# Chlumsky/msdfgen

Hardware: AMD Instinct MI355X
Metric: MSDF glyphs/sec (64x64, fp32) (higher is better)
Workload: dtype f64

## Files before the change

### msdfgen_amd/csrc/msdf_capi.hip

```cpp

#include <hip/hip_runtime.h>

#include <atomic>
#include <chrono>
#include <condition_variable>
#include <cmath>
#include <cstdarg>
#include <cstdio>
#include <cstdlib>
#include <cstring>
#include <deque>
#include <functional>
#include <memory>
#include <mutex>
#include <string>
#include <thread>
#include <vector>

#include <sched.h>

#include "msdf_kernels.hpp"
#include "msdf_single.hpp"

using namespace msdfhip;
// ... 18 lines not shown

static long long nowNsEarly() { return std::chrono::duration_cast<std::chrono::nanoseconds>(std::chrono::steady_clock::now().time_since_epoch()).count(); }

struct Tuning {
    size_t resLdsBudget;
    long persistentRounds;
    bool serialClasses;
    int querySlotCap, queryLpcContours;
    bool hasQueryLds;
    bool hasQueryPolicy;
    int qpEdgeCost, qpMaxEdges, qpMinCount, qpWideMaxEdges;
    float qpWideLoad, qpWideMeanCount;
    size_t signCap;
    bool pipelineTrace;
    int microbatch;
    int queryStatic;
    int queryGridSteps;
    int queryBatch;
    bool noArgPayloadSingle;
    bool noZeroCopySingle;
    bool noFusedSingle;
    double shareGridFactor;
    long persistentGrid;
    long shortRounds;
    long smallLaunchTiles;
    char devices[256];
    int smallMaxEdges;
    int ldsClassTpw;
    int pipelineDepth;
    bool prepLargeTier;
    int hostThreads;
    long singleSpinLimit;
    bool singleVerbose;
};
std::atomic<const Tuning *> gTuning(NULL);
std::mutex gTuningMutex;
std::vector<Tuning *> gTuningTables;

void readTuning() {
    Tuning &t = *new Tuning;
    const char *env;
    t.resLdsBudget = (env = getenv("MSDFHIP_RES_LDS_BUDGET")) ? (size_t) atol(env) : (size_t) 10*1024;
    t.persistentRounds = (env = getenv("MSDFHIP_PERSISTENT_ROUNDS")) ? atol(env) : 8;
    t.serialClasses = getenv("MSDFHIP_SERIAL_CLASSES") != NULL;
    t.querySlotCap = 160, t.queryLpcContours = 24;
    t.hasQueryLds = (env = getenv("MSDFHIP_QUERY_LDS")) != NULL;
    if (env)
        sscanf(env, "%d,%d", &t.querySlotCap, &t.queryLpcContours);
    t.qpEdgeCost = 150, t.qpMaxEdges = 48, t.qpMinCount = 0x7fffffff, t.qpWideMaxEdges = 128, t.qpWideLoad = 4e8f, t.qpWideMeanCount = 24.f;
    t.hasQueryPolicy = (env = getenv("MSDFHIP_QUERY_POLICY")) != NULL;
    if (env)
        sscanf(env, "%d,%d,%d,%d,%f,%f", &t.qpEdgeCost, &t.qpMaxEdges, &t.qpMinCount, &t.qpWideMaxEdges, &t.qpWideLoad, &t.qpWideMeanCount);
    t.signCap = (env = getenv("MSDFHIP_SIGN_CAP")) ? (size_t) atol(env) : (size_t) 192;
    if (t.signCap < 3)
        t.signCap = 3;
    t.pipelineTrace = getenv("MSDFHIP_PIPELINE_TRACE") != NULL;
    t.microbatch = (env = getenv("MSDFHIP_MICROBATCH")) ? atoi(env) : 256;
    if (t.microbatch < 1)
        t.microbatch = 1;
    t.devices[0] = 0;
    t.queryStatic = (env = getenv("MSDFHIP_QUERY_STATIC")) ? atoi(env) : 2;
    t.queryGridSteps = (env = getenv("MSDFHIP_QUERY_GRID")) ? atoi(env) : 16;
    t.queryBatch = (env = getenv("MSDFHIP_QUERY_BATCH")) && atoi(env) > 0 ? atoi(env) : 1;
    t.noFusedSingle = getenv("MSDFHIP_NO_FUSED_SINGLE") != NULL;
    t.noZeroCopySingle = getenv("MSDFHIP_NO_ZERO_COPY_SINGLE") != NULL;
    t.noArgPayloadSingle = getenv("MSDFHIP_NO_ARG_PAYLOAD_SINGLE") != NULL;
    t.shortRounds = (env = getenv("MSDFHIP_SHORT_ROUNDS")) ? atol(env) : 4;
    t.persistentGrid = (env = getenv("MSDFHIP_PERSISTENT_GRID")) ? atol(env) : 0;
    t.shareGridFactor = (env = getenv("MSDFHIP_SHARE_GRID")) ? atof(env) : 1.33;
    t.smallLaunchTiles = (env = getenv("MSDFHIP_SMALL_LAUNCH_TILES")) ? atol(env) : 8192;
    if ((env = getenv("MSDFHIP_DEVICES")))
        snprintf(t.devices, sizeof(t.devices), "%s", env);
    t.smallMaxEdges = (env = getenv("MSDFHIP_SMALL_MAX_EDGES")) && atoi(env) > 0 ? atoi(env) : 128;
    t.ldsClassTpw = (env = getenv("MSDFHIP_LDS_CLASS_TPW")) && atoi(env) == 1 ? 1 : 4;
    t.pipelineDepth = (env = getenv("MSDFHIP_PIPELINE_DEPTH")) && atoi(env) >= 1 && atoi(env) <= 3 ? atoi(env) : 2;
    t.prepLargeTier = getenv("MSDFHIP_PREP_LARGE_TIER") != NULL;
    t.hostThreads = (env = getenv("MSDFHIP_HOST_THREADS")) && atoi(env) > 0 ? atoi(env) : 0;
    t.singleSpinLimit = (env = getenv("MSDFHIP_SINGLE_SPIN_LIMIT")) && atol(env) > 0 ? atol(env) : 0;
    t.singleVerbose = getenv("MSDFHIP_SINGLE_VERBOSE") != NULL;
    gTuningTables.push_back(&t);
    gTuning.store(&t, std::memory_order_release);
}

const Tuning &tuning() {
    const Tuning *t = gTuning.load(std::memory_order_acquire);
    if (!t) {
        std::lock_guard<std::mutex> lock(gTuningMutex);
        if (!gTuning.load(std::memory_order_acquire))
            readTuning();
        t = gTuning.load(std::memory_order_acquire);
    }
    return *t;
}

std::atomic<unsigned long long> gRouteCounts[MSDFHIP_ROUTE_COUNT];

inline void countRoute(int route) { gRouteCounts[route].fetch_add(1, std::memory_order_relaxed); }

#define HIPCHK(expr) do { hipError_t e_ = (expr); if (e_ != hipSuccess) { (void) hipGetLastError(); return fail(MSDFHIP_ERR_HIP, "%s failed: %s (%s:%d)", #expr, hipGetErrorString(e_), __FILE__, __LINE__); } } while (0)

int ensureDevice(int dev = -1) {
    if (gDevice.load() < 0) {
        int rc = msdfhip_init(0);
        if (rc != MSDFHIP_OK)
            return rc;
    }
    if (dev < 0)
        dev = gDevice.load();
    else if (dev != gDevice.load()) {
        static std::atomic<unsigned long long> checked(0);
        if (dev >= 64 || !((checked.load()>>dev)&1ull)) {
            hipDeviceProp_t prop;
// ... 661 lines not shown
        } else if (rc == MSDFHIP_OK)
            rc = counted(launchDistance<SEL, false, false>(b, dGlyphs, w, h, dst, toScratch, simple, sOne, b->dBucket, b->nOne), MSDFHIP_ROUTE_DIST_ONE_QUAD);
    }
    hipError_t joinError = hipSuccess;
    if (sRest != stream) {
        hipError_t e = hipEventRecord(b->joinEvent[0], sRest);
        if (e == hipSuccess)
            e = hipStreamWaitEvent(stream, b->joinEvent[0], 0);
        joinError = e != hipSuccess ? e : joinError;
    }
    if (sOne != stream) {
        hipError_t e = hipEventRecord(b->joinEvent[1], sOne);
        if (e == hipSuccess)
            e = hipStreamWaitEvent(stream, b->joinEvent[1], 0);
        joinError = e != hipSuccess ? e : joinError;
    }
    rc = aheadRc != MSDFHIP_OK ? aheadRc : rc;
    if (joinError != hipSuccess) {
        (void) hipGetLastError();
        if (sRest != stream)
            (void) hipStreamSynchronize(sRest);
        if (sOne != stream)
            (void) hipStreamSynchronize(sOne);
        if (rc == MSDFHIP_OK)
            rc = fail(MSDFHIP_ERR_HIP, "joining the glyph-class streams failed: %s", hipGetErrorString(joinError));
    }
    if (rc == MSDFHIP_OK && nHuge > 0)
        rc = launchUnculled<SEL, true>(b, dGlyphs, w, h, dst, toScratch, stream, b->dBucket+nCulled, nHuge);
    return rc;
}

size_t candidateRecords(int nGlyphs, size_t texelsPerGlyph) { return ecHeaderRecords(nGlyphs)+(size_t) nGlyphs*ecSegment(texelsPerGlyph); }
size_t offsetRecords(int nGlyphs) { return (ecOffsetInts(nGlyphs)*sizeof(int)+sizeof(EcCandidate)-1)/sizeof(EcCandidate); }
size_t deferredRecords(int nGlyphs, size_t texelsPerGlyph, int nEdges) {
    return candidateRecords(nGlyphs, texelsPerGlyph)+offsetRecords(nGlyphs)+((size_t) (nEdges > 0 ? nEdges : 1)*2*sizeof(int)+sizeof(EcCandidate)-1)/sizeof(EcCandidate);
}

int ensureDeferred(const MsdfHipBatch *b, size_t cap, EcCandidate **out) {
    std::lock_guard<std::mutex> lock(b->scratchMutex);
    if (b->deferredCap < cap) {
        if (b->dDeferred)
            hipFree(b->dDeferred);
        b->dDeferred = NULL;
        b->deferredCap = 0;
        HIPCHK(hipMalloc((void **) &b->dDeferred, cap*sizeof(EcCandidate)));
        b->deferredCap = cap;
    }
    if (!b->dEcParams)
        HIPCHK(hipMalloc((void **) &b->dEcParams, sizeof(EcGlyphParams)*(size_t) (b->nGlyphs > b->glyphCap ? b->nGlyphs : b->glyphCap > 0 ? b->glyphCap : 1)));
    *out = b->dDeferred;
    return MSDFHIP_OK;
}

template <int N, bool OVERLAP>
unsigned queryResidentBlocks(int device, size_t lds) {
    enum { LDS_STEP = 2048, LDS_STEPS = 81 };
    static std::atomic<int> cache[LDS_STEPS];
    const size_t step = (lds+LDS_STEP-1)/LDS_STEP;
    if (step >= LDS_STEPS)
        return 0;
    int v = cache[step].load();
    if (!v) {
        int perCu = 0;
        if (hipOccupancyMaxActiveBlocksPerMultiprocessor(&perCu, reinterpret_cast<const void *>(k_ec_query<N, OVERLAP>), WAVE, step*LDS_STEP) != hipSuccess) {
            (void) hipGetLastError();
            perCu = 0;
        }
        v = perCu > 0 ? perCu*residentSlots(device) : -1;
// ... 46 lines not shown
    bool wideSlots = false;
    if (b->nGlyphs < 256 && !tuning().hasQueryLds) {
        const int wide = b->maxEdges < 1024 ? (b->maxEdges > 0 ? b->maxEdges : 1) : 1024;
        const int wideMerged = b->maxContours < wide ? (b->maxContours > 0 ? b->maxContours : 1) : wide;
        if ((size_t) b->maxContours*sizeof(double)+(size_t) (wide+wideMerged)*sizeof(PBSlot) <= (size_t) 64*1024 && wide > slotCap)
            slotCap = wide, wideSlots = true;
    }
    EcQueryPolicy lpcMaxContours;
    lpcMaxContours.lpcMaxContours = b->maxContours < lpcContoursWanted ? b->maxContours : lpcContoursWanted;
    lpcMaxContours.lpcEdgeCost = tuning().qpEdgeCost, lpcMaxContours.lpcMaxEdges = tuning().qpMaxEdges, lpcMaxContours.lpcMinCount = tuning().qpMinCount;
    lpcMaxContours.wideMaxEdges = tuning().qpWideMaxEdges, lpcMaxContours.wideLoad = tuning().qpWideLoad, lpcMaxContours.wideMeanCount = tuning().qpWideMeanCount;
    lpcMaxContours.gridSteps = tuning().queryGridSteps;
    const size_t resLanes = OVERLAP ? (size_t) (lpcMaxContours.lpcMaxContours > 0 ? lpcMaxContours.lpcMaxContours : 1)*WAVE*sizeof(double) : 0;
    const int slotOffset = OVERLAP ? (b->maxContours > 0 ? b->maxContours : 1) : 0;
    const int mergedCap = b->maxContours < slotCap ? (b->maxContours > 0 ? b->maxContours : 1) : slotCap;
    const size_t coopLds = (size_t) slotOffset*sizeof(double)+(size_t) (slotCap+mergedCap)*sizeof(PBSlot);
    const size_t queryLds = resLanes > coopLds ? resLanes : coopLds;
    const size_t fastLds = ecFastLdsBytes(b->maxEdges, N);
    if (GRES && queryLds > (size_t) gLdsLimit.load() && fastLds <= (size_t) gLdsLimit.load()) {
        if (paramsOnly)
            return MSDFHIP_OK;
        hipLaunchKernelGGL((k_ec_slow<N, OVERLAP, GRES>), dim3(slowGrid), dim3(WAVE), slowLds, stream, viewOf(b), dGlyphs, w, h, src, out, stencil, cfg,
                           (const EcCandidate *) NULL, 0u, 0, gres, gresStride);
        HIPCHK(hipGetLastError());
        countRoute(MSDFHIP_ROUTE_EC_SLOW_ALL);
        return MSDFHIP_OK;
    }
    if (fastLds > (size_t) gLdsLimit.load() || queryLds > (size_t) gLdsLimit.load())
        return fail(MSDFHIP_ERR_TOO_COMPLEX, "a glyph has %d contours / %d edges: the error-correction pass needs %zu B of LDS per wavefront, device limit is %d B",
                    b->maxContours, b->maxEdges, fastLds > queryLds ? fastLds : queryLds, gLdsLimit.load());
    rc = setLds(k_ec_query<N, OVERLAP>, queryLds);
    if (rc != MSDFHIP_OK)
        return rc;
    rc = setLds(k_ec_fast<N>, fastLds);
    if (rc != MSDFHIP_OK)
        return rc;
    int *offsets = reinterpret_cast<int *>(deferred+candidateRecords(b->nGlyphs, (size_t) w*h));
    int *corners = reinterpret_cast<int *>(deferred+candidateRecords(b->nGlyphs, (size_t) w*h)+offsetRecords(b->nGlyphs));
    const size_t wanted = allTexels/512;
    unsigned queryBlocks = (unsigned) (wanted < 64 ? 64 : wanted > 8192 ? 8192 : wanted);
    const bool staticDeal = tuning().queryStatic != 0;
    if (staticDeal) {
        const unsigned resident = queryResidentBlocks<N, OVERLAP>(b->device, queryLds);
        if (resident && queryBlocks > resident)
            queryBlocks = resident;
    }
    if (!call.ecParamsQueued)
        hipLaunchKernelGGL(k_ec_params, dim3((unsigned) b->nGlyphs), dim3(WAVE), 0, stream, b->dEcParams, viewOf(b), dGlyphs, cfg,
                           reinterpret_cast<unsigned *>(deferred), corners, offsets+ecSizesAt(b->nGlyphs));
    const int *ecOrder = NULL;
    rc = ensureEcOrder(b, &ecOrder, stream);
    if (rc != MSDFHIP_OK)
        return rc;
    if (paramsOnly) {
        HIPCHK(hipGetLastError());
        call.ecParamsQueued = true;
        return MSDFHIP_OK;
    }
    hipLaunchKernelGGL((k_ec_fast<N>), dim3(blocks), dim3(WAVE), fastLds, stream, viewOf(b), dGlyphs, w, h, tilesX, tiles, src, out, stencil, cfg,
                       (const EcGlyphParams *) b->dEcParams, deferred, seg, b->maxEdges, (const int *) corners);
    hipLaunchKernelGGL(k_ec_scan, dim3(1), dim3(1024), 0, stream, b->nGlyphs, reinterpret_cast<const unsigned *>(deferred), seg, offsets, lpcMaxContours, ecOrder);
    hipLaunchKernelGGL((k_ec_query<N, OVERLAP>), dim3(queryBlocks), dim3(WAVE), queryLds, stream, b->nGlyphs, b->dGlyphContourOffsets, b->dContourOffsets,
                       (const EdgeRec *) viewOf(b).recs, viewOf(b).windings, dGlyphs, w, h, src, out, stencil, cfg,
                       (const EcGlyphParams *) b->dEcParams, (const EcCandidate *) deferred, seg, (const int *) offsets, offsets+2*(size_t) b->nGlyphs+2, tuning().queryBatch, slotCap, slotOffset, lpcMaxContours,
                       call.overflowOut, ecOrder, staticDeal ? (tuning().queryStatic == 2 ? 5 : 1) : 0);
    if (call.overflowOut)
        call.overflowMirrored = true;
    else
        hipLaunchKernelGGL((k_ec_slow<N, OVERLAP, GRES>), dim3(slowGrid), dim3(WAVE), slowLds, stream, viewOf(b), dGlyphs, w, h, src, out, stencil, cfg,
                           (const EcCandidate *) deferred, seg, 1, gres, gresStride);
    HIPCHK(hipGetLastError());
    countRoute(ecOrder ? MSDFHIP_ROUTE_EC_QUERY_HEAVIEST : MSDFHIP_ROUTE_EC_QUERY_BATCH);
    if (wideSlots)
        countRoute(MSDFHIP_ROUTE_EC_WIDE_SLOTS);
    return MSDFHIP_OK;
}

template <int N>
int dispatchEc(const MsdfHipBatch *b, const MsdfHipGlyph *dGlyphs, int w, int h, const float *src, float *out, uint8_t *stencil,
               const MsdfHipConfig &cfg, hipStream_t stream, GenerateCall &call, bool paramsOnly) {
    if (!cfg.overlap_support)
        return launchEc<N, false, false>(b, dGlyphs, w, h, src, out, stencil, cfg, stream, call, paramsOnly);
    const bool globalRes = (size_t) b->maxContours*WAVE*sizeof(double) > 96*1024;
    return globalRes ? launchEc<N, true, true>(b, dGlyphs, w, h, src, out, stencil, cfg, stream, call, paramsOnly)
                     : launchEc<N, true, false>(b, dGlyphs, w, h, src, out, stencil, cfg, stream, call, paramsOnly);
}

int checkConfig(const MsdfHipConfig *cfg) {
    if (!cfg)
        return fail(MSDFHIP_ERR_INVALID, "cfg is NULL");
    if (cfg->ec_mode < 0 || cfg->ec_mode > 3 || cfg->ec_distance_check < 0 || cfg->ec_distance_check > 2 || cfg->ec_stage_limit < 0 || cfg->ec_stage_limit > 4)
        return fail(MSDFHIP_ERR_INVALID, "bad error-correction config (mode %d, distance check %d, stage limit %d)", cfg->ec_mode, cfg->ec_distance_check, cfg->ec_stage_limit);
    return MSDFHIP_OK;
// ... 3001 lines not shown
```

### msdfgen_amd/csrc/msdf_ec_fast.hpp

```cpp
#pragma once

#include "msdf_ec.hpp"

namespace msdfhip {

enum { EC_DEFER = 0x80 };

MSDF_HD bool ecHasBasePass(const EcParams &p) { return p.distanceCheck == EC_DO_NOT_CHECK || (p.distanceCheck == EC_CHECK_AT_EDGE && p.mode != EC_MODE_EDGE_ONLY); }
MSDF_HD bool ecHasShapePass(const EcParams &p) { return p.distanceCheck == EC_ALWAYS_CHECK || p.distanceCheck == EC_CHECK_AT_EDGE; }

struct FastCtx {
    double span;
    bool p1;
    bool pShape;
    bool basePass, shapePass;
};

MSDF_HD int rangeTest2(const FastCtx &c, double at, double bt, double xt, float am, float bm, float xm) {
    const bool inversion = (am > .5f && bm > .5f && xm <= .5f) || (am < .5f && bm < .5f && xm >= .5f);
    const bool outside = medianf(am, bm, xm) != xm;
    const bool candBase = c.basePass && (inversion || (!c.p1 && outside));
    const bool candShape = c.shapePass && (inversion || (!c.pShape && outside));
    if (!(candBase || candShape))
        return 0;
// ... 23 lines not shown
    const double s = flo > 0 ? 1. : -1.;
    const double as = a*s, bs = b*s, cs = c*s;
    if (as <= 0)
        return false;
    if (!(-bs > 2*as*lo*(1-1e-9) && -bs < 2*as*hi*(1+1e-9)))
        return false;
    return !(4*as*cs-bs*bs > 1e-9*mag*mag);
}

MSDF_HD bool bernsteinMayHaveRoot(float dA, float dBC, float dD) {
    const float m = fmaxf(fmaxf(fabsf(dA), fabsf(dBC)), fabsf(dD));
    const float eps = 1e-5f*m;
    const float h = .5f*dBC;
    return !((dA > eps && h > eps && dD > eps) || (dA < -eps && h < -eps && dD < -eps));
}

MSDF_HD bool edgeBetweenTexelsChannelFast(const float *a, const float *b, int channel) {
    const double n = a[channel]-.5;
    const double d = a[channel]-b[channel];
    if (!((n > 0 && d > 0 && n < d) || (n < 0 && d < 0 && n > d)))
        return false;
    const double t = n/d;
    if (t > 0 && t < 1) {
        float c[3] = { mixf(a[0], b[0], t), mixf(a[1], b[1], t), mixf(a[2], b[2], t) };
        return medianf(c[0], c[1], c[2]) == c[channel];
    }
    return false;
}

MSDF_HD int edgeBetweenTexelsFast(const float *a, const float *b) {
    return 1*(int) edgeBetweenTexelsChannelFast(a, b, 0)+2*(int) edgeBetweenTexelsChannelFast(a, b, 1)+4*(int) edgeBetweenTexelsChannelFast(a, b, 2);
}

template <class Sink>
MSDF_HD int diagonalPairFast(const FastCtx &cx, float am, float dm, const float *a, const float *l, const float *q,
                             float dA, float dBC, float dD, float l0, float q0, float l1, float q1, Sink &sink) {
    const double qa = dD-dBC+dA, qb = dBC-dA-dA, qc = dA;
    if (!quadraticMayHaveRootInRange(qa, qb, qc))
        return 0;
    double t[2];
    const int solutions = solveQuadratic(t, qa, qb, qc);
    int verdict = 0;
    for (int i = 0; i < solutions; ++i) {
        if (t[i] > MSDF_ARTIFACT_T_EPSILON && t[i] < 1-MSDF_ARTIFACT_T_EPSILON) {
            const float xm = interpolatedMedianQuad(a, l, q, t[i]);
            int rangeFlags = rangeTest2(cx, 0, 1, t[i], am, dm, xm);
            const double tEx0 = -.5*l0/q0, tEx1 = -.5*l1/q1;
            if (tEx0 > 0 && tEx0 < 1) {
                double tEnd0 = 0, tEnd1 = 1;
                float em0 = am, em1 = dm;
                const float ex = interpolatedMedianQuad(a, l, q, tEx0);
                if (tEx0 > t[i])
                    tEnd1 = tEx0, em1 = ex;
                else
                    tEnd0 = tEx0, em0 = ex;
                rangeFlags |= rangeTest2(cx, tEnd0, tEnd1, t[i], em0, em1, xm);
            }
            if (tEx1 > 0 && tEx1 < 1) {
                double tEnd0 = 0, tEnd1 = 1;
                float em0 = am, em1 = dm;
                const float ex = interpolatedMedianQuad(a, l, q, tEx1);
                if (tEx1 > t[i])
                    tEnd1 = tEx1, em1 = ex;
                else
                    tEnd0 = tEx1, em0 = ex;
                rangeFlags |= rangeTest2(cx, tEnd0, tEnd1, t[i], em0, em1, xm);
            }
            const int v = judge(rangeFlags);
            if (v&2)
                sink(t[i]);
            verdict |= v;
            if (verdict&1)
// ... 86 lines not shown
        if (!(cdev >= nb.dev[dy+1][dx+1]))
            continue;
        MSDF_UNROLL
        for (int j = 0; j < 3; ++j) {
            const int i0 = j, i1 = j == 2 ? 0 : j+1;
            const float dA = c[i1]-c[i0], dB = b[i1]-b[i0];
            if ((dA > 0 && dB < 0) || (dA < 0 && dB > 0))
                emit(k, j);
        }
    }
    MSDF_UNROLL
    for (int k = 4; k < 8; ++k) {
        const int dx = (k&1) ? 1 : -1, dy = (k&2) ? 1 : -1;
        if (!(nb.valid&(1u<<((dy+1)*3+(dx+1)))))
            continue;
        const float *d = nb.v[dy+1][dx+1];
        if (!(cdev >= nb.dev[dy+1][dx+1]))
            continue;
        const float *b = nb.v[1][dx+1], *cc = nb.v[dy+1][1];
        MSDF_UNROLL
        for (int j = 0; j < 3; ++j) {
            const int i0 = j, i1 = j == 2 ? 0 : j+1;
            const float dA = c[i1]-c[i0], dBC = b[i1]-b[i0]+cc[i1]-cc[i0], dD = d[i1]-d[i0];
            if (dA == 0 && dBC == 0 && dD == 0)
                continue;
            if (bernsteinMayHaveRoot(dA, dBC, dD))
                emit(k, j);
        }
    }
}

MSDF_HD float pick3(const float *v, int i) { return i == 0 ? v[0] : i == 1 ? v[1] : v[2]; }

template <class Sink>
MSDF_HD int evaluatePair(const float *c, const float *n, const float *hb, const float *vc, const EcParams &p, bool p1, int flip, int k, int j, Sink &sink) {
    FastCtx cx;
    cx.basePass = ecHasBasePass(p);
    cx.shapePass = ecHasShapePass(p);
    cx.p1 = p1;
    cx.pShape = (p.distanceCheck == EC_CHECK_AT_EDGE) ? true : p1;
    const int dx = ecNeighbourDx(k), dy = ecNeighbourDy(k);
    const int i0 = j, i1 = j == 2 ? 0 : j+1;
    const float cm = medianf(c[0], c[1], c[2]), nm = medianf(n[0], n[1], n[2]);
    if (k < 4) {
        cx.span = dy == 0 ? p.hSpan : p.vSpan;
        const float dA = pick3(c, i1)-pick3(c, i0), dB = pick3(n, i1)-pick3(n, i0);
        const double t = (double) dA/(dA-dB);
        if (t > MSDF_ARTIFACT_T_EPSILON && t < 1-MSDF_ARTIFACT_T_EPSILON) {
            const float xm = interpolatedMedianLin(c, n, t);
            const int v = judge(rangeTest2(cx, 0, 1, t, cm, nm, xm));
            if (v&2)
                sink(t, dx, flip ? -dy : dy);
            return v;
        }
        return 0;
    }
    cx.span = p.dSpan;
    const float *a = c, *b = hb, *cc = vc, *d = n;
    const float abc[3] = { a[0]-b[0]-cc[0], a[1]-b[1]-cc[1], a[2]-b[2]-cc[2] };
    const float l[3] = { -a[0]-abc[0], -a[1]-abc[1], -a[2]-abc[2] };
    const float q[3] = { d[0]+abc[0], d[1]+abc[1], d[2]+abc[2] };
    const float a3[3] = { a[0], a[1], a[2] };
    struct DirSink {
        Sink &sink;
        int dx, dy;
        MSDF_HD void operator()(double t) { sink(t, dx, dy); }
    } dirSink = { sink, dx, flip ? -dy : dy };
    const float dA = pick3(a, i1)-pick3(a, i0), dBC = pick3(b, i1)-pick3(b, i0)+pick3(cc, i1)-pick3(cc, i0), dD = pick3(d, i1)-pick3(d, i0);
    return diagonalPairFast(cx, cm, nm, a3, l, q, dA, dBC, dD, pick3(l, i0), pick3(q, i0), pick3(l, i1), pick3(q, i1), dirSink);
}

template <class Sink>
MSDF_HD int texelFindFast(const Neighbourhood &nb, const EcParams &p, bool p1, int flip, Sink &sink) {
    struct Items {
        unsigned char k[24], j[24];
        int n;
        MSDF_HD void operator()(int kk, int jj) { k[n] = (unsigned char) kk, j[n] = (unsigned char) jj; ++n; }
    } items;
    items.n = 0;
    texelCandidatePairs(nb, items);
    int verdict = 0;
    for (int i = 0; i < items.n; ++i) {
        const int k = items.k[i], dx = ecNeighbourDx(k), dy = ecNeighbourDy(k);
        verdict |= evaluatePair(nb.v[1][1], nb.v[dy+1][dx+1], nb.v[1][dx+1], nb.v[dy+1][1], p, p1, flip, k, items.j[i], sink);
    }
    return verdict;
}

template <class Sink>
MSDF_HD int ecTexelFast(const SdfView &sdf, const EcParams &p, const int *corners, int nCorners, int x, int yn, Sink &sink) {
    const int ys = sdf.flip ? sdf.h-1-yn : yn;
    Neighbourhood nb;
    loadNeighbourhood(nb, sdf, x, yn);
    int st = 0;
    if (p.mode == EC_MODE_EDGE_PRIORITY) {
        for (int i = 0; i < nCorners; ++i) {
            const int l = corners[2*i], b = corners[2*i+1];
            if ((x == l || x == l+1) && (ys == b || ys == b+1)) {
                st |= EC_PROTECTED;
                break;
            }
        }
// ... 34 lines not shown
```

### msdfgen_amd/csrc/msdf_kernels.hpp

```cpp
#pragma once

#include <hip/hip_runtime.h>
#include "msdf_device.hpp"
#include "msdf_prep.hpp"
#include "msdf_ec.hpp"
#include "msdf_ec_fast.hpp"
#include "msdf_cull.hpp"
#include "msdf_scanline.hpp"
#include "msdf_shapeprep.hpp"
#include "../../include/msdfgen_hip.h"

namespace msdfhip {

#ifndef MSDF_DISTANCE_WAVES_PER_SIMD
#define MSDF_DISTANCE_WAVES_PER_SIMD 4
#endif
constexpr int TILE = 8;
constexpr int WAVE = 64;
constexpr int REC_DOUBLES = sizeof(EdgeRec)/sizeof(double);

struct BatchView {
    int nGlyphs;
    const int32_t *glyphContourOffsets;
    const int32_t *contourOffsets;
// ... 908 lines not shown
            atomicAdd(&gQueryDetail[8], (unsigned long long) C), atomicAdd(&gQueryDetail[9], (unsigned long long) (slots ? 1 : 0));
        }
#endif
        return out[0];
    }
};

struct EcCandidate {
    unsigned texel;
    int dir;
    double t;
};
static_assert(sizeof(EcCandidate) == 16, "EcCandidate layout");

MSDF_HD size_t ecHeaderRecords(int nGlyphs) { return ((size_t) (nGlyphs+1)*sizeof(unsigned)+sizeof(EcCandidate)-1)/sizeof(EcCandidate); }
MSDF_HD unsigned ecSegment(size_t texelsPerGlyph) { return (unsigned) (texelsPerGlyph/8 > 64 ? (texelsPerGlyph/8+63)/64*64 : 64); }

struct CandidateSink {
    unsigned *header;
    EcCandidate *segment;
    unsigned seg, texel;
    int g;
    __device__ void operator()(double t, int dx, int dy) {
        const unsigned slot = atomicAdd(&header[1+g], 1u);
        if (slot < seg) {
            EcCandidate c;
            c.texel = texel, c.dir = (dx+1)|((dy+1)<<2), c.t = t;
            segment[slot] = c;
        } else
            header[0] = 1u;
    }
};

MSDF_HD size_t stencilIndex(size_t texel, int yn, int width, int height, int stencilYDown) {
    return stencilYDown ? texel+(size_t) (height-1-2*yn)*width : texel;
}

struct EcGlyphParams {
    double hSpan, vSpan, dSpan, texelX, texelY;
    float radiusH, radiusV, radiusD;
    int cornerBegin, nCorners;
    int pad;
};
static_assert(sizeof(EcGlyphParams) == 64, "EcGlyphParams layout");

__device__ __forceinline__ void ecParamsBody(EcGlyphParams *out, const BatchView &batch, const MsdfHipGlyph *glyphs, const MsdfHipConfig &cfg, unsigned *candidateHeader,
                                             int *corners, int *sizes, const int g, const int lane) {
    if (candidateHeader && lane == 0) {
        candidateHeader[1+g] = 0;
        if (g == 0)
            candidateHeader[0] = 0;
    }
    EcParams p;
    p.t = loadXform(glyphs[g]);
    p.minDeviationRatio = cfg.min_deviation_ratio;
    p.minImproveRatio = cfg.min_improve_ratio;
    ecDerive(p);
    const int c0 = batch.glyphContourOffsets[g], C = batch.glyphContourOffsets[g+1]-c0;
    const int e0 = batch.contourOffsets[c0], nE = batch.contourOffsets[c0+C]-e0;
    int nCorners = 0;
    if (cfg.ec_mode == EC_MODE_EDGE_PRIORITY && corners) {
        const EdgeRec *rec = batch.recs+e0;
        for (int base = 0; base < nE; base += WAVE) {
            const int e = base+lane;
            const bool corner = e < nE && (rec[e].flags&REC_CORNER);
            const unsigned long long mask = __ballot(corner);
            if (corner) {
                const V2 pp = project(p.t, ld(rec[e].p0));
                const int slot = e0+nCorners+__popcll(mask&((1ull<<lane)-1ull));
                corners[2*slot] = (int) floor(pp.x-.5);
                corners[2*slot+1] = (int) floor(pp.y-.5);
            }
            nCorners += __popcll(mask);
        }
    }
    if (lane == 0) {
        EcGlyphParams o;
        o.hSpan = p.hSpan, o.vSpan = p.vSpan, o.dSpan = p.dSpan, o.texelX = p.texelX, o.texelY = p.texelY;
        o.radiusH = p.radiusH, o.radiusV = p.radiusV, o.radiusD = p.radiusD, o.cornerBegin = e0, o.nCorners = nCorners, o.pad = 0;
        out[g] = o;
        if (sizes)
            sizes[2*g] = nE, sizes[2*g+1] = C;
    }
}
__global__ void __launch_bounds__(WAVE)
k_ec_params(EcGlyphParams *out, BatchView batch, const MsdfHipGlyph *glyphs, MsdfHipConfig cfg, unsigned *candidateHeader, int *corners, int *sizes) {
    ecParamsBody(out, batch, glyphs, cfg, candidateHeader, corners, sizes, (int) blockIdx.x, (int) threadIdx.x);
}

#ifndef MSDF_EC_FAST_WAVES_PER_SIMD
#define MSDF_EC_FAST_WAVES_PER_SIMD 7
#endif
enum { EC_HALO = TILE+2, EC_QUEUE_CAP = WAVE*24, EC_PROTECT_QUEUE_CAP = WAVE*8 };
__host__ __device__ inline size_t ecFastLdsBytes(int maxEdges, int n) {
    return (size_t) EC_HALO*EC_HALO*n*sizeof(float)+(WAVE+4)*sizeof(int)
           +(EC_QUEUE_CAP+EC_PROTECT_QUEUE_CAP)*sizeof(unsigned short);
}

template <int N>
__device__ __forceinline__ void ecFastBody(const BatchView &batch, const MsdfHipGlyph *glyphs, int width, int height, int tilesX, int tilesPerGlyph,
          const float *src, float *out, uint8_t *stencilOut, const MsdfHipConfig &cfg, const EcGlyphParams *glyphParams, EcCandidate *cands, unsigned seg,
          int maxEdges, const int *corners, const unsigned blockId, int *smemFast, const int sinkSlots = 0, const int sinkSlot = 0) {
    const GlyphWork wk = decodeItem(blockId, batch.nGlyphs, tilesPerGlyph);
    if (!wk.valid)
        return;
    float *halo = reinterpret_cast<float *>(smemFast);
    int *verdictLds = reinterpret_cast<int *>(halo+EC_HALO*EC_HALO*N);
    int *itemCount = verdictLds+WAVE;
    unsigned short *queue = reinterpret_cast<unsigned short *>(itemCount+4);
    unsigned short *protectQueue = queue+EC_QUEUE_CAP;
    float *devLds = reinterpret_cast<float *>(queue+EC_QUEUE_CAP)-EC_HALO*EC_HALO;
    static_assert((EC_QUEUE_CAP*sizeof(unsigned short))%sizeof(float) == 0 && EC_QUEUE_CAP*sizeof(unsigned short) >= EC_HALO*EC_HALO*sizeof(float), "devLds overlays the queue's tail");
    const int lane = threadIdx.x;
    const MsdfHipGlyph gd = glyphs[wk.g];
    EcParams p;
    p.t = loadXform(gd);
    p.minDeviationRatio = cfg.min_deviation_ratio;
    p.minImproveRatio = cfg.min_improve_ratio;
    p.mode = cfg.ec_mode, p.distanceCheck = cfg.ec_distance_check, p.overlap = cfg.overlap_support, p.stageLimit = 0;
    const EcGlyphParams gp = glyphParams[wk.g];
    p.hSpan = gp.hSpan, p.vSpan = gp.vSpan, p.dSpan = gp.dSpan, p.texelX = gp.texelX, p.texelY = gp.texelY;
    p.radiusH = gp.radiusH, p.radiusV = gp.radiusV, p.radiusD = gp.radiusD;
    const int tx = wk.tile%tilesX, ty = wk.tile/tilesX;

    const int lxT = lane&(TILE-1), lyT = lane>>3;
    const int xT = tx*TILE+lxT, ysT = gd.flip ? height-1-(ty*TILE+lyT) : ty*TILE+lyT;
    bool cornerTexel = false;
    if (p.mode == EC_MODE_EDGE_PRIORITY) {
        const int x0 = tx*TILE, x1 = tx*TILE+TILE-1;
        const int ya = gd.flip ? height-1-(ty*TILE+TILE-1) : ty*TILE, yb = gd.flip ? height-1-ty*TILE : ty*TILE+TILE-1;
        const int *list = corners+2*(size_t) gp.cornerBegin;
        for (int base = 0; base < gp.nCorners; base += WAVE) {
            const int k = base+lane;
            int l = 0, b = 0;
            bool near = false;
// ... 68 lines not shown
            int lane;
            __device__ void operator()(int k, int j) { queue[atomicAdd(count, 1)] = (unsigned short) (lane|k<<6|j<<9); }
        } push = { queue, itemCount, lane };
        texelCandidatePairs(nb, push);
    }
    verdictLds[lane] = (st&EC_PROTECTED) ? 0x100 : 0;
    waveSync();

    const int nProtect = itemCount[1];
    for (int base = 0; base < nProtect; base += WAVE) {
        const int it = base+lane;
        if (it >= nProtect)
            continue;
        const unsigned item = protectQueue[it];
        const int s = item&63, m = item>>6;
        const int sx = s&(TILE-1), sy = s>>3;
        const float *self = halo+((sy+1)*EC_HALO+sx+1)*N, *other = halo+((sy+m/3)*EC_HALO+sx+m%3)*N;
        if (evaluateProtectPair(self, other, m))
            atomicOr(&verdictLds[s], 0x100);
    }
    waveSync();

    const int nItems = itemCount[0];
    for (int base = 0; base < nItems; base += WAVE) {
        const int it = base+lane;
        if (it >= nItems)
            continue;
        const unsigned item = queue[it];
        const int s = item&63, k = (item>>6)&7, jp = item>>9;
        const int sx = s&(TILE-1), sy = s>>3;
        const int dx = ecNeighbourDx(k), dy = ecNeighbourDy(k);
        const float *c = halo+((sy+1)*EC_HALO+sx+1)*N, *n = halo+((sy+1+dy)*EC_HALO+sx+1+dx)*N;
        const float *hb = halo+((sy+1)*EC_HALO+sx+1+dx)*N, *vc = halo+((sy+1+dy)*EC_HALO+sx+1)*N;
        CandidateSink sink;
        sink.header = reinterpret_cast<unsigned *>(cands);
        sink.segment = sinkSlots > 0 ? cands+ecHeaderRecords(sinkSlots)+(size_t) sinkSlot*seg : cands+ecHeaderRecords(batch.nGlyphs)+(size_t) wk.g*seg;
        sink.seg = seg, sink.g = sinkSlots > 0 ? sinkSlot : wk.g;
        sink.texel = (unsigned) (((size_t) wk.g*height+ty*TILE+sy)*width+tx*TILE+sx);
        const int v = evaluatePair(c, n, hb, vc, p, (verdictLds[s]&0x100) != 0, gd.flip, k, jp, sink);
        if (v)
            atomicOr(&verdictLds[s], v);
    }
    waveSync();

    if (!inside)
        return;
    const int verdict = verdictLds[lane];
    if ((verdict&0x100) || (ecHasBasePass(p) && p.distanceCheck == EC_CHECK_AT_EDGE))
        st |= EC_PROTECTED;
    if (verdict&1)
        st |= EC_ERROR;
    const size_t texel = ((size_t) wk.g*height+yn)*width+x;
    const float *in = halo+((ly+1)*EC_HALO+lx+1)*N;
    float v[N];
    for (int i = 0; i < N; ++i)
        v[i] = in[i];
    if (st&EC_ERROR) {
        const float m = medianf(v[0], v[1], v[2]);
        v[0] = m, v[1] = m, v[2] = m;
    }
    float *px = out+gd.out_offset+(ptrdiff_t) gd.row_stride*yn+(ptrdiff_t) N*x;
    for (int i = 0; i < N; ++i)
        px[i] = v[i];
    if (stencilOut)
        stencilOut[stencilIndex(texel, yn, width, height, cfg.stencil_y_down)] = (uint8_t) st;
}
template <int N>
__global__ void __launch_bounds__(WAVE, MSDF_EC_FAST_WAVES_PER_SIMD)
k_ec_fast(BatchView batch, const MsdfHipGlyph *glyphs, int width, int height, int tilesX, int tilesPerGlyph,
          const float *src, float *out, uint8_t *stencilOut, MsdfHipConfig cfg, const EcGlyphParams *glyphParams, EcCandidate *cands, unsigned seg,
          int maxEdges, const int *corners) {
    extern __shared__ int smemFast[];
    ecFastBody<N>(batch, glyphs, width, height, tilesX, tilesPerGlyph, src, out, stencilOut, cfg, glyphParams, cands, seg, maxEdges, corners, blockIdx.x, smemFast);
}

struct EcQueryPolicy { int lpcMaxContours, lpcEdgeCost, lpcMaxEdges, lpcMinCount, wideMaxEdges; float wideLoad, wideMeanCount; int gridSteps; };
MSDF_HD int ecQueryGridSlices(unsigned count, int nE, int C, EcQueryPolicy q) {
    if (q.gridSteps <= 0 || C > q.lpcMaxContours || count == 0)
        return 0;
    int J = 1;
    while (J < (int) count && J < WAVE)
        J <<= 1;
    int S = WAVE/J, need = 1;
    while (need*q.gridSteps < nE && need < WAVE)
        need <<= 1;
    if (need > S)
        S = need;
    return S >= 2 && S <= WAVE/2 ? S : 0;
}
MSDF_HD bool ecQueryLanePerCandidate(unsigned count, int nE, int C, EcQueryPolicy q) {
    if (C > q.lpcMaxContours)
        return false;
    if ((nE > q.lpcMaxEdges && (int) count < q.lpcMinCount))
        return false;
    const long long coop = (long long) count*(340ll*((nE+WAVE-1)/WAVE)+10ll*nE+1000ll);
    const long long lpc = (long long) ((count+WAVE-1)/WAVE)*((long long) q.lpcEdgeCost*nE+1000ll);
    return lpc < coop;
}
MSDF_HD int ecQueryItems(unsigned count, unsigned seg, int nE, int C, EcQueryPolicy lpcMaxContours) {
    if (count > seg)
        return 0;
    const int S = ecQueryGridSlices(count, nE, C, lpcMaxContours);
    if (S)
        return (int) ((count+WAVE/S-1)/(WAVE/S));
    return ecQueryLanePerCandidate(count, nE, C, lpcMaxContours) ? (int) ((count+WAVE-1)/WAVE) : (int) count;
}
// ... 808 lines not shown
```

Baseline: 1.728 million.

## Defer expensive diagonal error-correction tails to a separate compacted kernel

The fast error-correction kernel now runs only a cheap root-existence prefilter on diagonal pairs. Surviving pairs on texels not already marked as errors are compacted into striped global lists via wave-aggregated atomics. A new k_ec_diag kernel prefix-sums the stripe counts and evaluates those tails densely, writing the median correction and stencil bit. The aim is to remove divergence from the costly quadratic-solve path inside the tile kernel, at the cost of an extra launch, global scratch, and reloading the field from memory, with in-kernel evaluation as the fallback when a stripe overflows.

```diff
diff --git a/msdfgen_amd/csrc/msdf_capi.hip b/msdfgen_amd/csrc/msdf_capi.hip
--- a/msdfgen_amd/csrc/msdf_capi.hip
+++ b/msdfgen_amd/csrc/msdf_capi.hip
@@ -74,6 +74,7 @@
     int hostThreads;
     long singleSpinLimit;
     bool singleVerbose;
+    long ecDiagCap;
 };
 std::atomic<const Tuning *> gTuning(NULL);
 std::mutex gTuningMutex;
@@ -120,6 +121,7 @@
     t.hostThreads = (env = getenv("MSDFHIP_HOST_THREADS")) && atoi(env) > 0 ? atoi(env) : 0;
     t.singleSpinLimit = (env = getenv("MSDFHIP_SINGLE_SPIN_LIMIT")) && atol(env) > 0 ? atol(env) : 0;
     t.singleVerbose = getenv("MSDFHIP_SINGLE_VERBOSE") != NULL;
+    t.ecDiagCap = (env = getenv("MSDFHIP_EC_DIAG_CAP")) ? (atol(env) > 0 ? atol(env) : 0) : -1;
     gTuningTables.push_back(&t);
     gTuning.store(&t, std::memory_order_release);
 }
@@ -847,8 +849,17 @@
 
 size_t candidateRecords(int nGlyphs, size_t texelsPerGlyph) { return ecHeaderRecords(nGlyphs)+(size_t) nGlyphs*ecSegment(texelsPerGlyph); }
 size_t offsetRecords(int nGlyphs) { return (ecOffsetInts(nGlyphs)*sizeof(int)+sizeof(EcCandidate)-1)/sizeof(EcCandidate); }
+size_t cornerRecords(int nEdges) { return ((size_t) (nEdges > 0 ? nEdges : 1)*2*sizeof(int)+sizeof(EcCandidate)-1)/sizeof(EcCandidate); }
+enum { EC_DIAG_PER_TILE = 32 };
+size_t ecDiagCapacity(int nGlyphs, size_t texelsPerGlyph) {
+    const long cap = tuning().ecDiagCap;
+    return cap >= 0 ? (size_t) cap : (size_t) nGlyphs*((texelsPerGlyph+TILE*TILE-1)/(TILE*TILE))*EC_DIAG_PER_TILE;
+}
+size_t diagRecords(size_t cap) {
+    return ((size_t) EC_DIAG_STRIPES*EC_DIAG_STRIDE*sizeof(unsigned)+(cap/EC_DIAG_STRIPES)*EC_DIAG_STRIPES*sizeof(EcDiagItem)+sizeof(EcCandidate)-1)/sizeof(EcCandidate);
+}
 size_t deferredRecords(int nGlyphs, size_t texelsPerGlyph, int nEdges) {
-    return candidateRecords(nGlyphs, texelsPerGlyph)+offsetRecords(nGlyphs)+((size_t) (nEdges > 0 ? nEdges : 1)*2*sizeof(int)+sizeof(EcCandidate)-1)/sizeof(EcCandidate);
+    return candidateRecords(nGlyphs, texelsPerGlyph)+offsetRecords(nGlyphs)+cornerRecords(nEdges)+diagRecords(ecDiagCapacity(nGlyphs, texelsPerGlyph));
 }
 
 int ensureDeferred(const MsdfHipBatch *b, size_t cap, EcCandidate **out) {
@@ -961,11 +972,17 @@
     rc = setLds(k_ec_query<N, OVERLAP>, queryLds);
     if (rc != MSDFHIP_OK)
         return rc;
-    rc = setLds(k_ec_fast<N>, fastLds);
+    rc = setLds(k_ec_fast<N, false>, fastLds);
+    if (rc == MSDFHIP_OK)
+        rc = setLds(k_ec_fast<N, true>, fastLds);
     if (rc != MSDFHIP_OK)
         return rc;
     int *offsets = reinterpret_cast<int *>(deferred+candidateRecords(b->nGlyphs, (size_t) w*h));
     int *corners = reinterpret_cast<int *>(deferred+candidateRecords(b->nGlyphs, (size_t) w*h)+offsetRecords(b->nGlyphs));
+    EcDiagList diag;
+    diag.counters = reinterpret_cast<unsigned *>(deferred+candidateRecords(b->nGlyphs, (size_t) w*h)+offsetRecords(b->nGlyphs)+cornerRecords(b->nEdges));
+    diag.stripeCap = (unsigned) (ecDiagCapacity(b->nGlyphs, (size_t) w*h)/EC_DIAG_STRIPES);
+    const bool deferDiag = ecDiagCapacity(b->nGlyphs, (size_t) w*h) > 0;
     const size_t wanted = allTexels/512;
     unsigned queryBlocks = (unsigned) (wanted < 64 ? 64 : wanted > 8192 ? 8192 : wanted);
     const bool staticDeal = tuning().queryStatic != 0;
@@ -976,7 +993,8 @@
     }
     if (!call.ecParamsQueued)
         hipLaunchKernelGGL(k_ec_params, dim3((unsigned) b->nGlyphs), dim3(WAVE), 0, stream, b->dEcParams, viewOf(b), dGlyphs, cfg,
-                           reinterpret_cast<unsigned *>(deferred), corners, offsets+ecSizesAt(b->nGlyphs));
+                           reinterpret_cast<unsigned *>(deferred), corners, offsets+ecSizesAt(b->nGlyphs),
+                           deferDiag ? diag.counters : (unsigned *) NULL);
     const int *ecOrder = NULL;
     rc = ensureEcOrder(b, &ecOrder, stream);
     if (rc != MSDFHIP_OK)
@@ -986,8 +1004,16 @@
         call.ecParamsQueued = true;
         return MSDFHIP_OK;
     }
-    hipLaunchKernelGGL((k_ec_fast<N>), dim3(blocks), dim3(WAVE), fastLds, stream, viewOf(b), dGlyphs, w, h, tilesX, tiles, src, out, stencil, cfg,
-                       (const EcGlyphParams *) b->dEcParams, deferred, seg, b->maxEdges, (const int *) corners);
+    if (deferDiag) {
+        hipLaunchKernelGGL((k_ec_fast<N, true>), dim3(blocks), dim3(WAVE), fastLds, stream, viewOf(b), dGlyphs, w, h, tilesX, tiles, src, out, stencil, cfg,
+                           (const EcGlyphParams *) b->dEcParams, deferred, seg, b->maxEdges, (const int *) corners, diag);
+        const size_t diagWanted = (size_t) residentSlots(b->device)*4u*8u*WAVE/EC_DIAG_BLOCK;
+        const unsigned diagBlocks = (unsigned) (blocks < (unsigned) EC_DIAG_STRIPES*4u ? (blocks+63u)/64u : diagWanted);
+        hipLaunchKernelGGL((k_ec_diag<N>), dim3(diagBlocks), dim3(EC_DIAG_BLOCK), 0, stream, b->nGlyphs, dGlyphs, w, h, src, out, stencil, cfg,
+                           (const EcGlyphParams *) b->dEcParams, deferred, seg, diag);
+    } else
+        hipLaunchKernelGGL((k_ec_fast<N, false>), dim3(blocks), dim3(WAVE), fastLds, stream, viewOf(b), dGlyphs, w, h, tilesX, tiles, src, out, stencil, cfg,
+                           (const EcGlyphParams *) b->dEcParams, deferred, seg, b->maxEdges, (const int *) corners, diag);
     hipLaunchKernelGGL(k_ec_scan, dim3(1), dim3(1024), 0, stream, b->nGlyphs, reinterpret_cast<const unsigned *>(deferred), seg, offsets, lpcMaxContours, ecOrder);
     hipLaunchKernelGGL((k_ec_query<N, OVERLAP>), dim3(queryBlocks), dim3(WAVE), queryLds, stream, b->nGlyphs, b->dGlyphContourOffsets, b->dContourOffsets,
                        (const EdgeRec *) viewOf(b).recs, viewOf(b).windings, dGlyphs, w, h, src, out, stencil, cfg,
diff --git a/msdfgen_amd/csrc/msdf_ec_fast.hpp b/msdfgen_amd/csrc/msdf_ec_fast.hpp
--- a/msdfgen_amd/csrc/msdf_ec_fast.hpp
+++ b/msdfgen_amd/csrc/msdf_ec_fast.hpp
@@ -79,12 +79,15 @@
     return 1*(int) edgeBetweenTexelsChannelFast(a, b, 0)+2*(int) edgeBetweenTexelsChannelFast(a, b, 1)+4*(int) edgeBetweenTexelsChannelFast(a, b, 2);
 }
 
-template <class Sink>
-MSDF_HD int diagonalPairFast(const FastCtx &cx, float am, float dm, const float *a, const float *l, const float *q,
+MSDF_HD bool diagonalPairMayHaveRoot(float dA, float dBC, float dD) {
+    const double qa = dD-dBC+dA, qb = dBC-dA-dA, qc = dA;
+    return quadraticMayHaveRootInRange(qa, qb, qc);
+}
+
+template <class Sink>
+MSDF_HD int diagonalPairTail(const FastCtx &cx, float am, float dm, const float *a, const float *l, const float *q,
                              float dA, float dBC, float dD, float l0, float q0, float l1, float q1, Sink &sink) {
     const double qa = dD-dBC+dA, qb = dBC-dA-dA, qc = dA;
-    if (!quadraticMayHaveRootInRange(qa, qb, qc))
-        return 0;
     double t[2];
     const int solutions = solveQuadratic(t, qa, qb, qc);
     int verdict = 0;
@@ -237,30 +240,23 @@
 
 MSDF_HD float pick3(const float *v, int i) { return i == 0 ? v[0] : i == 1 ? v[1] : v[2]; }
 
-template <class Sink>
-MSDF_HD int evaluatePair(const float *c, const float *n, const float *hb, const float *vc, const EcParams &p, bool p1, int flip, int k, int j, Sink &sink) {
+MSDF_HD bool diagonalMayNeedTail(const float *c, const float *n, const float *hb, const float *vc, int j) {
+    const int i0 = j, i1 = j == 2 ? 0 : j+1;
+    const float dA = pick3(c, i1)-pick3(c, i0), dBC = pick3(hb, i1)-pick3(hb, i0)+pick3(vc, i1)-pick3(vc, i0), dD = pick3(n, i1)-pick3(n, i0);
+    return diagonalPairMayHaveRoot(dA, dBC, dD);
+}
+
+template <class Sink>
+MSDF_HD int evaluateDiagonalTail(const float *c, const float *n, const float *hb, const float *vc, const EcParams &p, bool p1, int flip, int k, int j, Sink &sink) {
     FastCtx cx;
     cx.basePass = ecHasBasePass(p);
     cx.shapePass = ecHasShapePass(p);
     cx.p1 = p1;
     cx.pShape = (p.distanceCheck == EC_CHECK_AT_EDGE) ? true : p1;
+    cx.span = p.dSpan;
     const int dx = ecNeighbourDx(k), dy = ecNeighbourDy(k);
     const int i0 = j, i1 = j == 2 ? 0 : j+1;
     const float cm = medianf(c[0], c[1], c[2]), nm = medianf(n[0], n[1], n[2]);
-    if (k < 4) {
-        cx.span = dy == 0 ? p.hSpan : p.vSpan;
-        const float dA = pick3(c, i1)-pick3(c, i0), dB = pick3(n, i1)-pick3(n, i0);
-        const double t = (double) dA/(dA-dB);
-        if (t > MSDF_ARTIFACT_T_EPSILON && t < 1-MSDF_ARTIFACT_T_EPSILON) {
-            const float xm = interpolatedMedianLin(c, n, t);
-            const int v = judge(rangeTest2(cx, 0, 1, t, cm, nm, xm));
-            if (v&2)
-                sink(t, dx, flip ? -dy : dy);
-            return v;
-        }
-        return 0;
-    }
-    cx.span = p.dSpan;
     const float *a = c, *b = hb, *cc = vc, *d = n;
     const float abc[3] = { a[0]-b[0]-cc[0], a[1]-b[1]-cc[1], a[2]-b[2]-cc[2] };
     const float l[3] = { -a[0]-abc[0], -a[1]-abc[1], -a[2]-abc[2] };
@@ -272,7 +268,32 @@
         MSDF_HD void operator()(double t) { sink(t, dx, dy); }
     } dirSink = { sink, dx, flip ? -dy : dy };
     const float dA = pick3(a, i1)-pick3(a, i0), dBC = pick3(b, i1)-pick3(b, i0)+pick3(cc, i1)-pick3(cc, i0), dD = pick3(d, i1)-pick3(d, i0);
-    return diagonalPairFast(cx, cm, nm, a3, l, q, dA, dBC, dD, pick3(l, i0), pick3(q, i0), pick3(l, i1), pick3(q, i1), dirSink);
+    return diagonalPairTail(cx, cm, nm, a3, l, q, dA, dBC, dD, pick3(l, i0), pick3(q, i0), pick3(l, i1), pick3(q, i1), dirSink);
+}
+
+template <class Sink>
+MSDF_HD int evaluatePair(const float *c, const float *n, const float *hb, const float *vc, const EcParams &p, bool p1, int flip, int k, int j, Sink &sink) {
+    if (k >= 4)
+        return diagonalMayNeedTail(c, n, hb, vc, j) ? evaluateDiagonalTail(c, n, hb, vc, p, p1, flip, k, j, sink) : 0;
+    FastCtx cx;
+    cx.basePass = ecHasBasePass(p);
+    cx.shapePass = ecHasShapePass(p);
+    cx.p1 = p1;
+    cx.pShape = (p.distanceCheck == EC_CHECK_AT_EDGE) ? true : p1;
+    cx.span = ecNeighbourDy(k) == 0 ? p.hSpan : p.vSpan;
+    const int dx = ecNeighbourDx(k), dy = ecNeighbourDy(k);
+    const int i0 = j, i1 = j == 2 ? 0 : j+1;
+    const float cm = medianf(c[0], c[1], c[2]), nm = medianf(n[0], n[1], n[2]);
+    const float dA = pick3(c, i1)-pick3(c, i0), dB = pick3(n, i1)-pick3(n, i0);
+    const double t = (double) dA/(dA-dB);
+    if (t > MSDF_ARTIFACT_T_EPSILON && t < 1-MSDF_ARTIFACT_T_EPSILON) {
+        const float xm = interpolatedMedianLin(c, n, t);
+        const int v = judge(rangeTest2(cx, 0, 1, t, cm, nm, xm));
+        if (v&2)
+            sink(t, dx, flip ? -dy : dy);
+        return v;
+    }
+    return 0;
 }
 
 template <class Sink>
diff --git a/msdfgen_amd/csrc/msdf_kernels.hpp b/msdfgen_amd/csrc/msdf_kernels.hpp
--- a/msdfgen_amd/csrc/msdf_kernels.hpp
+++ b/msdfgen_amd/csrc/msdf_kernels.hpp
@@ -964,6 +964,18 @@
     }
 };
 
+enum { EC_DIAG_STRIPES = 256, EC_DIAG_STRIDE = 16, EC_DIAG_BLOCK = 256, EC_ITEM_TAIL = 0x8000 };
+struct EcDiagItem {
+    unsigned texel;
+    unsigned info;
+};
+static_assert(sizeof(EcDiagItem) == 8, "EcDiagItem layout");
+struct EcDiagList {
+    unsigned *counters;
+    unsigned stripeCap;
+    MSDF_HD EcDiagItem *items() const { return reinterpret_cast<EcDiagItem *>(counters+EC_DIAG_STRIPES*EC_DIAG_STRIDE); }
+};
+
 MSDF_HD size_t stencilIndex(size_t texel, int yn, int width, int height, int stencilYDown) {
     return stencilYDown ? texel+(size_t) (height-1-2*yn)*width : texel;
 }
@@ -977,12 +989,15 @@
 static_assert(sizeof(EcGlyphParams) == 64, "EcGlyphParams layout");
 
 __device__ __forceinline__ void ecParamsBody(EcGlyphParams *out, const BatchView &batch, const MsdfHipGlyph *glyphs, const MsdfHipConfig &cfg, unsigned *candidateHeader,
-                                             int *corners, int *sizes, const int g, const int lane) {
+                                             int *corners, int *sizes, const int g, const int lane, unsigned *diagCounters = NULL) {
     if (candidateHeader && lane == 0) {
         candidateHeader[1+g] = 0;
         if (g == 0)
             candidateHeader[0] = 0;
     }
+    if (diagCounters)
+        for (int stripe = g+lane*batch.nGlyphs; stripe < EC_DIAG_STRIPES; stripe += WAVE*batch.nGlyphs)
+            diagCounters[stripe*EC_DIAG_STRIDE] = 0;
     EcParams p;
     p.t = loadXform(glyphs[g]);
     p.minDeviationRatio = cfg.min_deviation_ratio;
@@ -1016,8 +1031,9 @@
     }
 }
 __global__ void __launch_bounds__(WAVE)
-k_ec_params(EcGlyphParams *out, BatchView batch, const MsdfHipGlyph *glyphs, MsdfHipConfig cfg, unsigned *candidateHeader, int *corners, int *sizes) {
-    ecParamsBody(out, batch, glyphs, cfg, candidateHeader, corners, sizes, (int) blockIdx.x, (int) threadIdx.x);
+k_ec_params(EcGlyphParams *out, BatchView batch, const MsdfHipGlyph *glyphs, MsdfHipConfig cfg, unsigned *candidateHeader, int *corners, int *sizes,
+            unsigned *diagCounters) {
+    ecParamsBody(out, batch, glyphs, cfg, candidateHeader, corners, sizes, (int) blockIdx.x, (int) threadIdx.x, diagCounters);
 }
 
 #ifndef MSDF_EC_FAST_WAVES_PER_SIMD
@@ -1029,10 +1045,11 @@
            +(EC_QUEUE_CAP+EC_PROTECT_QUEUE_CAP)*sizeof(unsigned short);
 }
 
-template <int N>
+template <int N, bool DIAG = false>
 __device__ __forceinline__ void ecFastBody(const BatchView &batch, const MsdfHipGlyph *glyphs, int width, int height, int tilesX, int tilesPerGlyph,
           const float *src, float *out, uint8_t *stencilOut, const MsdfHipConfig &cfg, const EcGlyphParams *glyphParams, EcCandidate *cands, unsigned seg,
-          int maxEdges, const int *corners, const unsigned blockId, int *smemFast, const int sinkSlots = 0, const int sinkSlot = 0) {
+          int maxEdges, const int *corners, const unsigned blockId, int *smemFast, const int sinkSlots = 0, const int sinkSlot = 0,
+          const EcDiagList diag = EcDiagList()) {
     const GlyphWork wk = decodeItem(blockId, batch.nGlyphs, tilesPerGlyph);
     if (!wk.valid)
         return;
@@ -1167,6 +1184,11 @@
         const int dx = ecNeighbourDx(k), dy = ecNeighbourDy(k);
         const float *c = halo+((sy+1)*EC_HALO+sx+1)*N, *n = halo+((sy+1+dy)*EC_HALO+sx+1+dx)*N;
         const float *hb = halo+((sy+1)*EC_HALO+sx+1+dx)*N, *vc = halo+((sy+1+dy)*EC_HALO+sx+1)*N;
+        if (DIAG && k >= 4) {
+            if (diagonalMayNeedTail(c, n, hb, vc, jp))
+                queue[it] = (unsigned short) (item|EC_ITEM_TAIL);
+            continue;
+        }
         CandidateSink sink;
         sink.header = reinterpret_cast<unsigned *>(cands);
         sink.segment = sinkSlots > 0 ? cands+ecHeaderRecords(sinkSlots)+(size_t) sinkSlot*seg : cands+ecHeaderRecords(batch.nGlyphs)+(size_t) wk.g*seg;
@@ -1177,6 +1199,50 @@
             atomicOr(&verdictLds[s], v);
     }
     waveSync();
+
+    if (DIAG) {
+        const unsigned stripe = blockId%EC_DIAG_STRIPES;
+        for (int base = 0; base < nItems; base += WAVE) {
+            const int it = base+lane;
+            unsigned item = 0;
+            bool tail = false;
+            if (it < nItems) {
+                item = queue[it];
+                tail = (item&EC_ITEM_TAIL) && !(verdictLds[item&63]&1);
+            }
+            const unsigned long long mask = __ballot(tail);
+            if (!mask)
+                continue;
+            unsigned first = 0;
+            if (lane == 0)
+                first = atomicAdd(diag.counters+stripe*EC_DIAG_STRIDE, (unsigned) __popcll(mask));
+            first = __builtin_amdgcn_readfirstlane(first);
+            if (!tail)
+                continue;
+            const unsigned slot = first+(unsigned) __popcll(mask&((1ull<<lane)-1ull));
+            const int s = item&63, k = (item>>6)&7, jp = (item>>9)&3;
+            const int sx = s&(TILE-1), sy = s>>3;
+            const bool p1 = (verdictLds[s]&0x100) != 0;
+            const unsigned texel = (unsigned) (((size_t) wk.g*height+ty*TILE+sy)*width+tx*TILE+sx);
+            if (slot < diag.stripeCap) {
+                EcDiagItem r;
+                r.texel = texel, r.info = (unsigned) (k-4)|(unsigned) jp<<2|(p1 ? 16u : 0u);
+                diag.items()[(size_t) stripe*diag.stripeCap+slot] = r;
+            } else {
+                const int dx = ecNeighbourDx(k), dy = ecNeighbourDy(k);
+                const float *c = halo+((sy+1)*EC_HALO+sx+1)*N, *n = halo+((sy+1+dy)*EC_HALO+sx+1+dx)*N;
+                const float *hb = halo+((sy+1)*EC_HALO+sx+1+dx)*N, *vc = halo+((sy+1+dy)*EC_HALO+sx+1)*N;
+                CandidateSink sink;
+                sink.header = reinterpret_cast<unsigned *>(cands);
+                sink.segment = cands+ecHeaderRecords(batch.nGlyphs)+(size_t) wk.g*seg;
+                sink.seg = seg, sink.g = wk.g, sink.texel = texel;
+                const int v = evaluateDiagonalTail(c, n, hb, vc, p, p1, gd.flip, k, jp, sink);
+                if (v)
+                    atomicOr(&verdictLds[s], v);
+            }
+        }
+        waveSync();
+    }
 
     if (!inside)
         return;
@@ -1200,13 +1266,99 @@
     if (stencilOut)
         stencilOut[stencilIndex(texel, yn, width, height, cfg.stencil_y_down)] = (uint8_t) st;
 }
-template <int N>
+template <int N, bool DIAG>
 __global__ void __launch_bounds__(WAVE, MSDF_EC_FAST_WAVES_PER_SIMD)
 k_ec_fast(BatchView batch, const MsdfHipGlyph *glyphs, int width, int height, int tilesX, int tilesPerGlyph,
           const float *src, float *out, uint8_t *stencilOut, MsdfHipConfig cfg, const EcGlyphParams *glyphParams, EcCandidate *cands, unsigned seg,
-          int maxEdges, const int *corners) {
+          int maxEdges, const int *corners, EcDiagList diag) {
     extern __shared__ int smemFast[];
-    ecFastBody<N>(batch, glyphs, width, height, tilesX, tilesPerGlyph, src, out, stencilOut, cfg, glyphParams, cands, seg, maxEdges, corners, blockIdx.x, smemFast);
+    ecFastBody<N, DIAG>(batch, glyphs, width, height, tilesX, tilesPerGlyph, src, out, stencilOut, cfg, glyphParams, cands, seg, maxEdges, corners, blockIdx.x, smemFast,
+                        0, 0, diag);
+}
+
+template <int N>
+__global__ void __launch_bounds__(EC_DIAG_BLOCK)
+k_ec_diag(int nGlyphs, const MsdfHipGlyph *__restrict__ glyphs, int width, int height, const float *__restrict__ src, float *__restrict__ out,
+          uint8_t *__restrict__ stencilOut, MsdfHipConfig cfg, const EcGlyphParams *__restrict__ glyphParams, EcCandidate *__restrict__ cands, unsigned seg,
+          EcDiagList diag) {
+    static_assert(EC_DIAG_BLOCK == EC_DIAG_STRIPES, "one stripe count per thread");
+    __shared__ unsigned prefix[EC_DIAG_STRIPES+1];
+    const int t = (int) threadIdx.x;
+    const unsigned count = diag.counters[t*EC_DIAG_STRIDE];
+    prefix[t+1] = count < diag.stripeCap ? count : diag.stripeCap;
+    if (t == 0)
+        prefix[0] = 0;
+    __syncthreads();
+    for (int off = 1; off < EC_DIAG_STRIPES; off <<= 1) {
+        const unsigned v = t >= off ? prefix[t+1-off] : 0u;
+        __syncthreads();
+        prefix[t+1] += v;
+        __syncthreads();
+    }
+    const unsigned total = prefix[EC_DIAG_STRIPES];
+    const unsigned texelsPerGlyph = (unsigned) width*(unsigned) height;
+    const unsigned stride = gridDim.x*EC_DIAG_BLOCK;
+    for (unsigned i0 = blockIdx.x*EC_DIAG_BLOCK+t; i0 < total; i0 += 2*stride) {
+        EcDiagItem r[2];
+        bool have[2];
+        MSDF_UNROLL
+        for (int u = 0; u < 2; ++u) {
+            const unsigned i = i0+u*stride;
+            have[u] = i < total;
+            if (have[u]) {
+                int lo = 0, hi = EC_DIAG_STRIPES-1;
+                while (lo < hi) {
+                    const int mid = (lo+hi+1)>>1;
+                    if (prefix[mid] <= i)
+                        lo = mid;
+                    else
+                        hi = mid-1;
+                }
+                r[u] = diag.items()[(size_t) lo*diag.stripeCap+(i-prefix[lo])];
+            }
+        }
+        float c[2][3], n[2][3], hb[2][3], vc[2][3];
+        int g[2], x[2], yn[2], k[2], jp[2], flip[2];
+        int64_t outOffset[2];
+        int rowStride[2];
+        double dSpan[2];
+        MSDF_UNROLL
+        for (int u = 0; u < 2; ++u) {
+            if (!have[u])
+                continue;
+            g[u] = (int) (r[u].texel/texelsPerGlyph);
+            const int rem = (int) (r[u].texel-(unsigned) g[u]*texelsPerGlyph);
+            yn[u] = rem/width, x[u] = rem%width;
+            k[u] = 4+(int) (r[u].info&3), jp[u] = (int) (r[u].info>>2)&3;
+            const int dx = ecNeighbourDx(k[u]), dy = ecNeighbourDy(k[u]);
+            const float *field = src+(size_t) g[u]*texelsPerGlyph*N;
+            const float *pc = field+((size_t) yn[u]*width+x[u])*N, *pn = field+((size_t) (yn[u]+dy)*width+x[u]+dx)*N;
+            const float *ph = field+((size_t) yn[u]*width+x[u]+dx)*N, *pv = field+((size_t) (yn[u]+dy)*width+x[u])*N;
+            for (int ch = 0; ch < 3; ++ch)
+                c[u][ch] = pc[ch], n[u][ch] = pn[ch], hb[u][ch] = ph[ch], vc[u][ch] = pv[ch];
+            flip[u] = glyphs[g[u]].flip, outOffset[u] = glyphs[g[u]].out_offset, rowStride[u] = glyphs[g[u]].row_stride;
+            dSpan[u] = glyphParams[g[u]].dSpan;
+        }
+        MSDF_UNROLL
+        for (int u = 0; u < 2; ++u) {
+            if (!have[u])
+                continue;
+            EcParams p;
+            p.mode = cfg.ec_mode, p.distanceCheck = cfg.ec_distance_check;
+            p.dSpan = dSpan[u];
+            CandidateSink sink;
+            sink.header = reinterpret_cast<unsigned *>(cands);
+            sink.segment = cands+ecHeaderRecords(nGlyphs)+(size_t) g[u]*seg;
+            sink.seg = seg, sink.g = g[u], sink.texel = r[u].texel;
+            if (evaluateDiagonalTail(c[u], n[u], hb[u], vc[u], p, (r[u].info&16) != 0, flip[u], k[u], jp[u], sink)&1) {
+                const float m = medianf(c[u][0], c[u][1], c[u][2]);
+                float *px = out+outOffset[u]+(ptrdiff_t) rowStride[u]*yn[u]+(ptrdiff_t) N*x[u];
+                px[0] = m, px[1] = m, px[2] = m;
+                if (stencilOut)
+                    stencilOut[stencilIndex(r[u].texel, yn[u], width, height, cfg.stencil_y_down)] |= (uint8_t) EC_ERROR;
+            }
+        }
+    }
 }
 
 struct EcQueryPolicy { int lpcMaxContours, lpcEdgeCost, lpcMaxEdges, lpcMinCount, wideMaxEdges; float wideLoad, wideMeanCount; int gridSteps; };
```

Result: no change. 1.739 million (median of 6 runs) (+0.6%).
